# mimoralea/gym-soccer-littman94

Hardware: AMD Instinct MI355X
Metric: env-steps/sec (whole node) at batch=1M random joint actions; HBM GB/s vs peak (higher is better)
Workload: dtype int8

## Files before the change

gym_soccer_littman94_amd/_lib.py:

```python
import ctypes as C
import os

_HERE = os.path.dirname(os.path.abspath(__file__))
LIB_PATH = os.path.join(_HERE, "libsoccer_hip.so")

OK, E_INVALID, E_HIP, E_NOMEM, E_STATE = 0, -1, -2, -3, -4
F_AUTORESET = 1
F_NULL_STREAM = 2
F_HOST_MAPPED = 4
F_STEP_STATS = 8
F_STREAM_ACTIONS = 16


class SoccerHipError(RuntimeError):
    """A HIP runtime failure inside libsoccer_hip.so."""


class Config(C.Structure):
    _fields_ = [("n_lanes", C.c_uint64), ("width", C.c_int32), ("height", C.c_int32),
                ("slip_prob", C.c_double), ("max_steps", C.c_int32), ("device", C.c_int32),
                ("seed", C.c_uint64), ("lane_offset", C.c_uint64), ("flags", C.c_uint32),
                ("envs_per_thread", C.c_uint32), ("stream", C.c_void_p)]


# ... 268 lines not shown
    "soccer_comm_unique_id": (C.c_int, [C.c_void_p]),
    "soccer_comm_init": (C.c_int, [C.c_void_p, C.c_int32, C.c_int32, C.c_void_p]),
    "soccer_comm_destroy": (C.c_int, [C.c_void_p]),
    "soccer_comm_all_gather": (C.c_int, [C.c_void_p, C.c_void_p, C.c_void_p, C.c_uint64]),
    "soccer_comm_sum_u64": (C.c_int, [C.c_void_p, C.c_void_p, C.c_int32]),
    "soccer_comm_max_f64": (C.c_int, [C.c_void_p, C.c_void_p, C.c_int32]),
    "soccer_comm_barrier": (C.c_int, [C.c_void_p]),
    "soccer_malloc": (C.c_int, [C.c_void_p, C.c_size_t, C.POINTER(C.c_void_p)]),
    "soccer_free": (C.c_int, [C.c_void_p, C.c_void_p]),
    "soccer_memcpy_h2d": (C.c_int, [C.c_void_p, C.c_void_p, C.c_void_p, C.c_size_t]),
    "soccer_memcpy_d2h": (C.c_int, [C.c_void_p, C.c_void_p, C.c_void_p, C.c_size_t]),
    "soccer_memset": (C.c_int, [C.c_void_p, C.c_void_p, C.c_int, C.c_size_t]),
    "soccer_timer_start": (C.c_int, [C.c_void_p]),
    "soccer_timer_stop": (C.c_int, [C.c_void_p, C.POINTER(C.c_float)]),
    "soccer_timer_mark": (C.c_int, [C.c_void_p]),
    "soccer_timer_read": (C.c_int, [C.c_void_p, C.POINTER(C.c_float)]),
    "soccer_stamp": (C.c_int, [C.c_void_p, C.c_int32]),
    "soccer_stamps_clear": (C.c_int, [C.c_void_p, C.c_int32, C.c_int32]),
    "soccer_stamps_read": (C.c_int, [C.c_void_p, C.c_int32, C.c_int32, C.c_void_p, C.POINTER(C.c_int32)]),
    "soccer_graph_begin": (C.c_int, [C.c_void_p]),
    "soccer_graph_end": (C.c_int, [C.c_void_p, C.POINTER(C.c_void_p)]),
    "soccer_graph_launch": (C.c_int, [C.c_void_p, C.c_void_p, C.c_int32]),
    "soccer_graph_info": (C.c_int, [C.c_void_p, C.POINTER(C.c_int32), C.POINTER(C.c_int64), C.POINTER(C.c_int32)]),
    "soccer_graph_destroy": (C.c_int, [C.c_void_p, C.c_void_p]),
}

_lib = None


def _share_torch_hip_runtime():
    import importlib.util
    import sys
    if os.environ.get("SOCCER_HIP_RUNTIME", "") == "system" or "torch" in sys.modules:
        return
    try:
        spec = importlib.util.find_spec("torch")
    except Exception:
        spec = None
    if spec is None or not spec.origin:
        return
    path = os.path.join(os.path.dirname(spec.origin), "lib", "libamdhip64.so")
    if os.path.exists(path):
        try:
            C.CDLL(path, mode=C.RTLD_GLOBAL)
        except OSError:
            pass
# ... 33 lines not shown
```

gym_soccer_littman94_amd/core.py:

```python
import ctypes as C
import weakref

import numpy as np

from . import _lib
from ._device import DeviceArray, _ptr
from ._lib import Config, RolloutArgs, StepArgs
from .learners import (GradientPlay, MinimaxQLearner, MinimaxQPopulation, OpponentModelPopulation, QLearner, QPopulation,
                       RegretLearner, RegretPopulation, WolfPHCLearner, WolfPopulation, _meta_of_cross_play, league_config,
                       minimax_q_config, minimax_q_population_config, om_derive, om_model, om_population_config, q_learning_config,
                       q_population_config, regret_average, regret_learner_config, regret_policy, regret_population_config,
                       wolf_phc_config, wolf_population_config)


def meta_lds_bytes(n_a, n_b):
    stride = (n_a + n_b + 2) | 1
    return 128 + 8 * ((n_a + 2) * stride + n_a + 1) + 4 * n_a


class SoccerBatch:

    def __init__(self, n_lanes, width=5, height=4, slip_prob=0.0, seed=0, autoreset=False,
                 max_steps=100, device=0, lane_offset=0, stream=None, envs_per_thread=0, host_mapped=False, step_stats=True,
                 stream_actions=False):
# ... 561 lines not shown
        self._check(self.lib.soccer_stamps_clear(self.h, int(first), int(count)))

    def stamps(self, first=0, count=256):
        t = np.zeros(int(count), np.uint64); khz = C.c_int32()
        self._check(self.lib.soccer_stamps_read(self.h, int(first), int(count), t.ctypes.data, C.byref(khz)))
        return t, int(khz.value)

    def graph_begin(self):
        self._check(self.lib.soccer_graph_begin(self.h))

    def graph_end(self):
        g = C.c_void_p()
        self._check(self.lib.soccer_graph_end(self.h, C.byref(g)))
        return g

    def graph_launch(self, g, replays=1):
        self._check(self.lib.soccer_graph_launch(self.h, g, int(replays)))

    def graph_info(self, g):
        nodes, steps, runs = C.c_int32(), C.c_int64(), C.c_int32()
        self._check(self.lib.soccer_graph_info(g, C.byref(nodes), C.byref(steps), C.byref(runs)))
        return {"kernel_nodes": int(nodes.value), "steps_fused": int(steps.value), "fused_launches": int(runs.value)}

    def graph_destroy(self, g):
        self.lib.soccer_graph_destroy(self.h, g)
```

gym_soccer_littman94_amd/csrc/soccer_handle.hpp:

```cpp
#pragma once
#include <hip/hip_runtime.h>

#include <string>
#include <vector>

#include "../../include/soccer_hip.h"
#include "soccer_inlists.hpp"
#include "soccer_kernels.hpp"
#include "soccer_plan_io.hpp"
#include "soccer_rules.hpp"

#pragma GCC visibility push(hidden)

using namespace soccer;

int fail(soccer_handle* h, int code, const char* fmt, ...);

#define HIP_TRY(h, expr)                                                                         \
    do {                                                                                         \
        hipError_t e_ = (expr);                                                                  \
        if (e_ != hipSuccess)                                                                    \
            return fail((h), e_ == hipErrorOutOfMemory ? SOCCER_E_NOMEM : SOCCER_E_HIP,          \
                        "%s failed: %s", #expr, hipGetErrorString(e_));                          \
    } while (0)

// ... 29 lines not shown
    void release(void* p) {
        for (size_t i = 0; i < bufs.size(); ++i) if (bufs[i].ptr == p) { drop(bufs[i]); bufs.erase(bufs.begin() + i); return; }
    }
    void clear() {
        for (const Buf& b : bufs) drop(b);
        bufs.clear(); ready = false;
    }

private:
    template <class T> static size_t bytes(size_t count) { return count ? count * sizeof(T) : 1; }
    static void drop(const Buf& b) { (void)(b.pinned ? hipHostFree(b.ptr) : hipFree(b.ptr)); }
    template <class T>
    int take(soccer_handle* h, hipError_t e, bool pinned, T** out) {
        if (e != hipSuccess) {
            *out = nullptr;
            return e == hipErrorOutOfMemory ? fail(h, SOCCER_E_NOMEM, "out of %s memory for %s", pinned ? "pinned host" : "device", what)
                                            : fail(h, SOCCER_E_HIP, "allocation for %s failed: %s", what, hipGetErrorString(e));
        }
        bufs.push_back(Buf{*out, pinned});
        return SOCCER_OK;
    }
};

struct soccer_graph {
    hipGraph_t graph = nullptr;
    hipGraphExec_t exec = nullptr;
    uint64_t ticks = 0;
    int start_slot = 0;
    bool stamped = false;
    int32_t kernel_nodes = 0;
    int64_t steps_fused = 0;
    int32_t fused_launches = 0;
};

struct PendingRun {
    soccer_step_args first{};
    int64_t len = 0;
    int64_t act_stride = 0, out_stride = 0;
};

struct Learner;

struct PassBufs {
    double* buf[2] = {nullptr, nullptr};
    unsigned long long* words = nullptr;
    int32_t* done = nullptr;
    int32_t* open = nullptr;
    int stride = 0;
};
// ... 38 lines not shown
    unsigned long long* d_hist = nullptr;
    unsigned int* d_misuse = nullptr;
    unsigned int* misuse_host = nullptr;
    uint8_t* d_state = nullptr;
    size_t state_stride = 0;
    int state_streams = 6;
    uint8_t* stage_dev = nullptr;
    uint8_t* stage_host = nullptr;
    bool mapped = false;
    size_t stage_bytes = 0;
    int tick_slot = 0;
    uint64_t tick = 0;
    bool slip = false, lut_lds = false;
    size_t smem_bytes = 0;
    int E = 4;
    int grid_cap = 2048;
    bool capturing = false;
    uint64_t capture_ticks = 0;
    int capture_calls = 0;
    int capture_start_slot = 0;
    PendingRun run;
    bool graph_fuse = true;
    int capture_kernels = 0;
    int64_t capture_steps_fused = 0; int capture_fused_launches = 0;
    int n_cu = 256;
    size_t lds_limit = 64 * 1024;
    uint4* d_sub = nullptr;
    uint4* rec_host = nullptr; uint4* rec_dev = nullptr; uint32_t rec_seq = 0;
    swar::Consts swar_c{}; bool swar_ok = false;
    swar::SlipConsts slip_c{}; bool slip_swar_ok = false;
    uint32_t* d_slip_lut = nullptr;
    uint32_t* d_slip_step_lut = nullptr;
    size_t hist_slots = kHistSlots;
    bool timer_stamped = false; int wall_clock_khz = 100000;
    bool capture_stamped = false;
    bool stamp_poll = false;
    unsigned long long stamp_prev = 0;
    unsigned long long swar_launch_lanes = kSwarLaunchLanes;
    int rollout_pref = 0;
    soccer_rollout_shape_info last_rollout{};
    SlipF64* d_slip_f64 = nullptr;
    uint32_t* d_worklist = nullptr;
    unsigned long long* d_traj_hist = nullptr;
    void* comm = nullptr; int comm_world = 0, comm_rank = 0;
    unsigned long long* d_comm_scratch = nullptr;
    PlanIO plan{};
// ... 27 lines not shown
    size_t mg_need[5] = {0, 0, 0, 0, 0};
    OwnedBufs mg_bufs{"the meta-game solver"};
    std::vector<Learner*> learners;
    std::string err;

    soccer_handle() = default;
    soccer_handle(const soccer_handle&) = delete;
    soccer_handle& operator=(const soccer_handle&) = delete;
    ~soccer_handle();
};

constexpr size_t kStampStride = 8;
constexpr size_t kMappedBytes = 64 + 8 * kStampStride * SOCCER_STAMP_SLOTS;

static inline void bind_tick(soccer_handle* h, KernelParams& P, uint64_t ticks) {
    P.tick_in = h->d_tick + (h->tick_slot ? 16 : 0);
    P.tick_out = h->d_tick + (h->tick_slot ? 0 : 16);
    h->tick_slot ^= 1;
    if (h->capturing) { h->capture_ticks += ticks; h->capture_calls += 1; }
    else h->tick += ticks;
}

static inline void note_kernel(soccer_handle* h) { if (h->capturing) h->capture_kernels += 1; }

static inline int grid_for(const soccer_handle* h, uint64_t work_items) {
    uint64_t blocks = (work_items + kBlock - 1) / kBlock;
    if (blocks < 1) blocks = 1;
    if (blocks > (uint64_t)h->grid_cap) blocks = h->grid_cap;
    return static_cast<int>(blocks);
}

hipError_t rollout_raise_smem_limit(const soccer_handle* h, size_t bytes);
int rollout_enqueue(soccer_handle* h, const soccer_rollout_args* a, const soccer_rollout_extra* x, unsigned long long* hist);
int flush_run(soccer_handle* h);
static inline int flush_pending(soccer_handle* h) { return h->run.len ? flush_run(h) : SOCCER_OK; }
void comm_release(soccer_handle* h);
void learners_release(soccer_handle* h);
void gradient_players_release(soccer_handle* h);
constexpr int kMinimaxBatch = 16;
int minimax_check(soccer_handle* h, const char* what, double gamma);
int minimax_prepare(soccer_handle* h);
int response_rows(soccer_handle* h, const char* what, const char* name, int n, const double* pol);
int response_upload(soccer_handle* h, double* dst, const double* pol, int n, hipMemcpyKind kind = hipMemcpyHostToDevice);

#pragma GCC visibility pop
```

gym_soccer_littman94_amd/csrc/soccer_hip.hip:

```cpp
#include <hip/hip_runtime.h>

#include <algorithm>
#include <atomic>
#include <chrono>
#include <cstdarg>
#include <cstdio>
#include <cstdlib>
#include <cstring>
#include <memory>
#include <string>
#include <vector>

#include "soccer_dispatch.hpp"
#include "soccer_handle.hpp"
#include "soccer_env_kernels.hpp"
#include "soccer_slip.hpp"

static thread_local std::string g_err;

int fail(soccer_handle* h, int code, const char* fmt, ...) {
    char buf[512];
    va_list ap; va_start(ap, fmt); vsnprintf(buf, sizeof buf, fmt, ap); va_end(ap);
    if (h) h->err = buf; else g_err = buf;
    return code;
// ... 125 lines not shown
        }
        if (ST.lut_step_ok && !std::getenv("SOCCER_STEP_SLIP_ONE_BY_ONE")) {
            std::vector<uint32_t> img(kSlipStepLdsWords, 0xFFFFFFFFu);
            std::memcpy(img.data(), ST.lut_step, kSlipStepBuckets);
            std::memcpy(img.data() + kSlipStepBuckets / 4, ST.T, sizeof(ST.T));
            if (int rc = h->bufs.alloc(nullptr, img.size(), &h->d_slip_step_lut)) return rc;
            HIP_TRY(nullptr, hipMemcpy(h->d_slip_step_lut, img.data(), img.size() * sizeof(uint32_t), hipMemcpyHostToDevice));
        }
        {
            const SlipF64 F = make_slip_f64(ST);
            if (int rc = h->bufs.alloc(nullptr, 1, &h->d_slip_f64)) return rc;
            HIP_TRY(nullptr, hipMemcpy(h->d_slip_f64, &F, sizeof F, hipMemcpyHostToDevice));
        }
        h->slip_c = swar::SlipConsts{};
        for (int i = 0; i < 9; ++i) h->slip_c.CB[i] = ST.CB[i];
        h->slip_c.c_off = ST.c_off;
    }
    set_key(h, cfg->seed);
    h->swar_ok = swar::fits(R.H, R.W, cfg->max_steps);
    if (h->swar_ok) h->swar_c = swar::make_consts(R.H, R.W, R.goal_lo, R.goal_hi, cfg->max_steps, R.n_isd, R.isd, P.autoreset != 0u);
    h->slip = cfg->slip_prob != 0.0;
    if (const char* e2 = std::getenv("SOCCER_ROLLOUT")) h->rollout_pref = std::atoi(e2);
    if (const char* e4 = std::getenv("SOCCER_GRAPH_FUSE")) h->graph_fuse = std::atoi(e4) != 0;
    if (const char* e3 = std::getenv("SOCCER_SWAR_LAUNCH_LANES")) {
        const unsigned long long v = std::strtoull(e3, nullptr, 10) & ~3ull;
        if (v >= 4ull && v <= kSwarLaunchLanes) h->swar_launch_lanes = v;
    }
    h->E = e ? static_cast<int>(e) : 4;

    const size_t nc_bytes = (R.next_cell.size() + kIsdWords) * sizeof(uint32_t);
    const size_t lut_bytes = R.lut.size() * sizeof(uint16_t);
    if (nc_bytes > 150 * 1024)
        return fail(nullptr, SOCCER_E_INVALID, "pitch too large: the move/bounds table (%zu bytes) must fit the 160 KB LDS", nc_bytes);
    if (int rc = h->bufs.alloc(nullptr, R.lut.size(), &h->d_lut)) return rc;
    HIP_TRY(nullptr, hipMemcpy(h->d_lut, R.lut.data(), lut_bytes, hipMemcpyHostToDevice));
    P.lut = h->d_lut; P.lut_len = static_cast<int32_t>(R.lut.size());
    h->lut_lds = nc_bytes + lut_bytes <= 150 * 1024;
    h->smem_bytes = nc_bytes + (h->lut_lds ? lut_bytes : 0);
    if (h->smem_bytes > 48 * 1024) {
        const size_t b = h->smem_bytes;
        hipError_t se = rollout_raise_smem_limit(h, b);
        if (se == hipSuccess)
            se = with_shape(h, [&](auto slip, auto lds) {
                return hipFuncSetAttribute(reinterpret_cast<const void*>(&reset_kernel<decltype(lds)::value, decltype(slip)::value>),
                                           hipFuncAttributeMaxDynamicSharedMemorySize, (int)b);
            });
// ... 46 lines not shown
    unsigned long long slots[32] = {0};
    slots[0] = tick; slots[16] = tick;
    HIP_TRY(h, hipMemcpy(h->d_tick, slots, sizeof slots, hipMemcpyHostToDevice));
    h->tick = tick;
    return SOCCER_OK;
}
extern "C" uint64_t soccer_get_seed(const soccer_handle* h) { return h ? h->cfg.seed : 0; }

extern "C" int batched_reset(soccer_handle* h, const uint8_t* mask, const double* u_reset, uint16_t* obs) {
    if (!h) return fail(nullptr, SOCCER_E_INVALID, "handle is NULL");
    if (!aligned(u_reset, 8) || !aligned(obs, 2))
        return fail(h, SOCCER_E_INVALID, "batched_reset: u_reset must be 8-byte and obs 2-byte aligned");
    HIP_TRY(h, hipSetDevice(h->cfg.device));
    if (int rc = flush_pending(h)) return rc;
    KernelParams P = h->P;
    bind_tick(h, P, 1);
    ResetIO io{mask, u_reset, obs};
    const ResetPlan R = plan_reset(handle_facts(h), ResetCall{mask != nullptr, u_reset != nullptr, aligned(mask, 4) && aligned(obs, 8)});
    const unsigned long long n4 = R.n4;
    if (n4) {
        ResetSwar RS{h->swar_c, P.state, P.state_stride, P.state_layout, n4, P.lane_offset, P.tick_in, P.tick_out, P.key0, P.key1, mask, obs};
        const dim3 g(static_cast<unsigned>(((n4 >> 2) + kBlock - 1) / kBlock)), b(kBlock);
        with_flag(R.masked, [&](auto masked) { with_flag(R.slip, [&](auto slip) {
            hipLaunchKernelGGL((reset_kernel_swar<decltype(masked)::value, decltype(slip)::value>), g, b, 0, h->stream, RS);
        }); });
        note_kernel(h);
    }
    if (n4 < P.n) {
        KernelParams Q = P;
        Q.first = n4; Q.n = P.n - n4;
        if (n4) Q.tick_out = nullptr;
        const dim3 g(grid_for(h, Q.n)), b(kBlock);
        with_flag(R.lut_lds, [&](auto lds) { with_flag(R.slip, [&](auto slip) {
            hipLaunchKernelGGL((reset_kernel<decltype(lds)::value, decltype(slip)::value>), g, b, h->smem_bytes, h->stream, Q, io);
        }); });
        note_kernel(h);
    }
    HIP_TRY(h, hipGetLastError());
    return SOCCER_OK;
}

static int fetch_state(soccer_handle* h, std::vector<uint8_t>& img) {
    const size_t n = h->P.n, S = h->state_stride, bytes = (size_t)h->state_streams * S;
    if (h->mapped) std::memcpy(img.data(), h->d_state, bytes);
    else HIP_TRY(h, hipMemcpy(img.data(), h->d_state, bytes, hipMemcpyDeviceToHost));
    if (h->state_streams == 3) {
        for (size_t i = 0; i < n; ++i) {
            swar::Group G;
            swar::unpack3(img[i], img[S + i], img[2 * S + i], G);
            img[5 * S + i] = (uint8_t)G.tt; img[4 * S + i] = (uint8_t)G.ps; img[3 * S + i] = (uint8_t)G.cb;
            img[2 * S + i] = (uint8_t)G.rb; img[S + i] = (uint8_t)G.ca; img[i] = (uint8_t)G.ra;
        }
    }
    return SOCCER_OK;
}

extern "C" int soccer_state_streams(const soccer_handle* h) { return h ? h->state_streams : 0; }
// ... 347 lines not shown
    if (hist) {
        std::vector<unsigned long long> shards(h->hist_slots * kHistStride);
        HIP_TRY(h, hipMemcpy(shards.data(), h->d_hist, shards.size() * sizeof(unsigned long long), hipMemcpyDeviceToHost));
        hist[0] = hist[1] = hist[2] = 0;
        for (size_t s = 0; s < h->hist_slots; ++s) for (int b = 0; b < 3; ++b) hist[b] += shards[s * kHistStride + b];
    }
    if (misuse) {
        const volatile unsigned int* m = h->misuse_host;
        *misuse = (m[0] ? 1u : 0u) | (m[1] ? 2u : 0u) | (m[2] ? 4u : 0u);
    }
    return SOCCER_OK;
}

extern "C" uint32_t soccer_peek_misuse(const soccer_handle* h) {
    if (!h || !h->misuse_host) return 0u;
    const volatile unsigned int* m = h->misuse_host;
    return (m[0] ? SOCCER_MISUSE_FROZEN : 0u) | (m[1] ? SOCCER_MISUSE_ACTION : 0u) | (m[2] ? SOCCER_MISUSE_OBSERVATION : 0u);
}

extern "C" int soccer_reset_stats(soccer_handle* h) {
    if (!h) return fail(nullptr, SOCCER_E_INVALID, "handle is NULL");
    HIP_TRY(h, hipSetDevice(h->cfg.device));
    if (int rc = flush_pending(h)) return rc;
    HIP_TRY(h, hipMemsetAsync(h->d_hist, 0, sizeof(unsigned long long) * h->hist_slots * kHistStride, h->stream));
    HIP_TRY(h, hipMemsetAsync(h->d_misuse, 0, 64, h->stream));
    return SOCCER_OK;
}

extern "C" int soccer_malloc(soccer_handle* h, size_t bytes, void** dptr) {
    if (!h || !dptr) return fail(h, SOCCER_E_INVALID, "handle/dptr is NULL");
    HIP_TRY(h, hipSetDevice(h->cfg.device));
    HIP_TRY(h, hipMalloc(dptr, bytes ? bytes : 1));
    return SOCCER_OK;
}
extern "C" int soccer_free(soccer_handle* h, void* dptr) {
    if (!h) return fail(nullptr, SOCCER_E_INVALID, "handle is NULL");
    HIP_TRY(h, hipSetDevice(h->cfg.device));
    if (dptr) HIP_TRY(h, hipFree(dptr));
    return SOCCER_OK;
}
extern "C" int soccer_memcpy_h2d(soccer_handle* h, void* dst, const void* src, size_t bytes) {
    if (!h) return fail(nullptr, SOCCER_E_INVALID, "handle is NULL");
    if (h->capturing) return fail(h, SOCCER_E_STATE, "soccer_memcpy_h2d during graph capture");
    HIP_TRY(h, hipSetDevice(h->cfg.device));
    HIP_TRY(h, hipMemcpyAsync(dst, src, bytes, hipMemcpyHostToDevice, h->stream));
    HIP_TRY(h, hipStreamSynchronize(h->stream));
    return SOCCER_OK;
}
extern "C" int soccer_memcpy_d2h(soccer_handle* h, void* dst, const void* src, size_t bytes) {
    if (!h) return fail(nullptr, SOCCER_E_INVALID, "handle is NULL");
    if (h->capturing) return fail(h, SOCCER_E_STATE, "soccer_memcpy_d2h during graph capture");
    HIP_TRY(h, hipSetDevice(h->cfg.device));
    HIP_TRY(h, hipMemcpyAsync(dst, src, bytes, hipMemcpyDeviceToHost, h->stream));
    HIP_TRY(h, hipStreamSynchronize(h->stream));
    return SOCCER_OK;
}
extern "C" int soccer_memset(soccer_handle* h, void* dst, int value, size_t bytes) {
    if (!h) return fail(nullptr, SOCCER_E_INVALID, "handle is NULL");
    HIP_TRY(h, hipSetDevice(h->cfg.device));
    if (int rc = flush_pending(h)) return rc;
    HIP_TRY(h, hipMemsetAsync(dst, value, bytes, h->stream));
    return SOCCER_OK;
}

__global__ void stamp_kernel(unsigned long long* slot) {
    if (threadIdx.x == 0) *slot = wall_clock64();
}

static volatile unsigned long long* stamp_host(soccer_handle* h) {
    return reinterpret_cast<volatile unsigned long long*>(reinterpret_cast<uint8_t*>(h->misuse_host) + 64);
}
static unsigned long long* stamp_dev(soccer_handle* h) {
    return reinterpret_cast<unsigned long long*>(reinterpret_cast<uint8_t*>(h->d_misuse) + 64);
}

extern "C" int soccer_stamp(soccer_handle* h, int32_t slot) {
    if (!h) return fail(nullptr, SOCCER_E_INVALID, "handle is NULL");
    if (slot < 0 || slot >= SOCCER_STAMP_SLOTS) return fail(h, SOCCER_E_INVALID, "stamp slot %d out of range (0..%d)", slot, SOCCER_STAMP_SLOTS - 1);
    HIP_TRY(h, hipSetDevice(h->cfg.device));
    if (int rc = flush_pending(h)) return rc;
    hipLaunchKernelGGL(stamp_kernel, dim3(1), dim3(64), 0, h->stream, stamp_dev(h) + kStampStride * slot);
    HIP_TRY(h, hipGetLastError());
    return SOCCER_OK;
}

extern "C" int soccer_stamps_clear(soccer_handle* h, int32_t first, int32_t count) {
    if (!h) return fail(nullptr, SOCCER_E_INVALID, "handle is NULL");
    if (first < 0 || count < 0 || first + count > SOCCER_STAMP_SLOTS) return fail(h, SOCCER_E_INVALID, "stamp range out of bounds");
    for (int32_t i = 0; i < count; ++i) stamp_host(h)[kStampStride * (first + i)] = 0ull;
    std::atomic_thread_fence(std::memory_order_seq_cst);
    return SOCCER_OK;
}

extern "C" int soccer_stamps_read(soccer_handle* h, int32_t first, int32_t count, uint64_t* ticks, int32_t* khz) {
    if (!h) return fail(nullptr, SOCCER_E_INVALID, "handle is NULL");
    if (first < 0 || count < 0 || first + count > SOCCER_STAMP_SLOTS || (count && !ticks)) return fail(h, SOCCER_E_INVALID, "stamp range out of bounds");
    for (int32_t i = 0; i < count; ++i) ticks[i] = stamp_host(h)[kStampStride * (first + i)];
    if (khz) *khz = h->wall_clock_khz;
    return SOCCER_OK;
}

extern "C" int soccer_timer_start(soccer_handle* h) {
    if (!h) return fail(nullptr, SOCCER_E_INVALID, "handle is NULL");
// ... 54 lines not shown
        __builtin_ia32_pause();
    }
    (void)hipGetLastError();
    HIP_TRY(h, hipEventElapsedTime(elapsed_ms, h->ev0, h->ev1));
    return SOCCER_OK;
}
extern "C" int soccer_timer_stop(soccer_handle* h, float* elapsed_ms) {
    if (int rc = soccer_timer_mark(h)) return rc;
    return soccer_timer_read(h, elapsed_ms);
}

__global__ void move_tick_kernel(unsigned long long* dst, const unsigned long long* src) {
    if (threadIdx.x == 0) *dst = *src;
}

extern "C" int soccer_graph_begin(soccer_handle* h) {
    if (!h) return fail(nullptr, SOCCER_E_INVALID, "handle is NULL");
    if (h->capturing) return fail(h, SOCCER_E_STATE, "graph capture already in progress");
    HIP_TRY(h, hipSetDevice(h->cfg.device));
    HIP_TRY(h, hipStreamBeginCapture(h->stream, hipStreamCaptureModeThreadLocal));
    h->capturing = true; h->capture_ticks = 0; h->capture_calls = 0; h->capture_stamped = false;
    h->capture_start_slot = h->tick_slot;
    h->run = PendingRun{}; h->capture_kernels = 0; h->capture_steps_fused = 0; h->capture_fused_launches = 0;
    return SOCCER_OK;
}

extern "C" int soccer_graph_end(soccer_handle* h, soccer_graph** out) {
    if (!h || !out) return fail(h, SOCCER_E_INVALID, "handle/out is NULL");
    if (!h->capturing) return fail(h, SOCCER_E_STATE, "no graph capture in progress");
    if (const int rc = flush_pending(h)) {
        const std::string why = h->err;
        hipGraph_t dead = nullptr;
        h->capturing = false; h->tick_slot = h->capture_start_slot;
        (void)hipStreamEndCapture(h->stream, &dead);
        if (dead) (void)hipGraphDestroy(dead);
        (void)hipGetLastError();
        h->err = why;
        return rc;
    }
    if (h->capture_calls % 2 != 0) {
        hipLaunchKernelGGL(move_tick_kernel, dim3(1), dim3(64), 0, h->stream,
                           h->d_tick + (h->capture_start_slot ? 16 : 0), h->d_tick + (h->tick_slot ? 16 : 0));
        h->tick_slot = h->capture_start_slot;
    }
    h->capturing = false;
    hipGraph_t graph = nullptr;
    HIP_TRY(h, hipStreamEndCapture(h->stream, &graph));
    soccer_graph* g = new soccer_graph();
    g->kernel_nodes = h->capture_kernels; g->steps_fused = h->capture_steps_fused; g->fused_launches = h->capture_fused_launches;
    g->graph = graph; g->ticks = h->capture_ticks; g->start_slot = h->capture_start_slot; g->stamped = h->capture_stamped;
    hipError_t e = hipGraphInstantiate(&g->exec, graph, nullptr, nullptr, 0);
    if (e != hipSuccess) {
        (void)hipGraphDestroy(graph); delete g;
        return fail(h, SOCCER_E_HIP, "hipGraphInstantiate failed: %s", hipGetErrorString(e));
    }
    (void)hipGraphUpload(g->exec, h->stream);
    (void)hipGetLastError();
    *out = g;
    return SOCCER_OK;
}

extern "C" int soccer_graph_launch(soccer_handle* h, soccer_graph* g, int32_t replays) {
    if (!h || !g) return fail(h, SOCCER_E_INVALID, "handle/graph is NULL");
    if (h->capturing) return fail(h, SOCCER_E_STATE, "soccer_graph_launch during graph capture");
    HIP_TRY(h, hipSetDevice(h->cfg.device));
    if (replays > 0 && h->tick_slot != g->start_slot) {
        HIP_TRY(h, hipMemcpyAsync(h->d_tick + (g->start_slot ? 16 : 0), h->d_tick + (h->tick_slot ? 16 : 0),
                                  sizeof(unsigned long long), hipMemcpyDeviceToDevice, h->stream));
        h->tick_slot = g->start_slot;
    }
    h->stamp_poll = replays == 1 && g->stamped && hipStreamQuery(h->stream) == hipSuccess;
    (void)hipGetLastError();
    h->timer_stamped = g->stamped;
    if (h->stamp_poll) h->stamp_prev = stamp_host(h)[kStampStride];
    for (int32_t r = 0; r < replays; ++r) HIP_TRY(h, hipGraphLaunch(g->exec, h->stream));
    h->tick += g->ticks * (uint64_t)(replays > 0 ? replays : 0);
    return SOCCER_OK;
}

extern "C" int soccer_graph_info(const soccer_graph* g, int32_t* kernel_nodes, int64_t* steps_fused, int32_t* fused_launches) {
    if (!g) return fail(nullptr, SOCCER_E_INVALID, "graph is NULL");
    if (kernel_nodes) *kernel_nodes = g->kernel_nodes;
    if (steps_fused) *steps_fused = g->steps_fused;
    if (fused_launches) *fused_launches = g->fused_launches;
    return SOCCER_OK;
}

extern "C" int soccer_graph_destroy(soccer_handle* h, soccer_graph* g) {
    if (!g) return SOCCER_OK;
    if (h) { (void)hipSetDevice(h->cfg.device); (void)hipStreamSynchronize(h->stream); }
    if (g->exec) (void)hipGraphExecDestroy(g->exec);
    if (g->graph) (void)hipGraphDestroy(g->graph);
    delete g;
    return SOCCER_OK;
}

extern "C" int soccer_trajectory_returns(soccer_handle* h, int32_t n_steps, const int8_t* reward, const uint8_t* terminated,
                                         const uint8_t* truncated, int64_t stride, int8_t* last_return,
                                         int32_t* episode_count, uint64_t hist[3]) {
    if (!h) return fail(nullptr, SOCCER_E_INVALID, "handle is NULL");
    if (h->capturing) return fail(h, SOCCER_E_STATE, "soccer_trajectory_returns during graph capture");
    if (n_steps < 1 || !reward || !terminated || !truncated)
        return fail(h, SOCCER_E_INVALID, "soccer_trajectory_returns: n_steps >= 1 and the reward / terminated / truncated trajectories are required");
    if (stride < (int64_t)h->P.n) return fail(h, SOCCER_E_INVALID, "soccer_trajectory_returns: stride must be >= n_lanes");
    if (!aligned(episode_count, 4)) return fail(h, SOCCER_E_INVALID, "soccer_trajectory_returns: episode_count must be 4-byte aligned");
    HIP_TRY(h, hipSetDevice(h->cfg.device));
    const size_t slots = (size_t)h->grid_cap * 2;
// ... 28 lines not shown
```

gym_soccer_littman94_amd/csrc/soccer_launch_plan.hpp:

```cpp
#pragma once
#include <cstddef>
#include <cstdint>

#include "../../include/soccer_hip.h"

namespace soccer {

struct HandleFacts {
    bool swar_ok, slip, slip_swar_ok;
    bool slip_lut, slip_step_lut;
    bool small, wide;
    bool lut_lds;
    bool policy_a, policy_b, step_stats, slip_int_one, stream_actions;
    bool capturing, worklist;
    int E, rollout_pref, nS;
    unsigned lane_phase;
    size_t smem_bytes, lds_limit;
    unsigned long long n;
};

struct StepCall {
    bool dword_io;
    bool u_step, u_reset, u_aligned16;
    bool last_return, last_return_aligned4;
// ... 143 lines not shown
    sh.full = R.full ? 1 : 0;
    sh.table_placement = R.table_placement;
    sh.parts = R.swar ? parts : 1; sh.chunks = chunks;
    sh.dynamic_lds_bytes = R.smem;
    return sh;
}

struct ResetCall {
    bool mask, u_reset, dword_io;
};

struct ResetPlan {
    unsigned long long n4;
    bool masked, slip, lut_lds;
};

inline ResetPlan plan_reset(const HandleFacts& f, const ResetCall& c) {
    ResetPlan R{};
    if (f.swar_ok && !c.u_reset && f.E != 1 && f.lane_phase == 0u && c.dword_io) R.n4 = f.n & ~3ull;
    R.masked = c.mask; R.slip = f.slip; R.lut_lds = f.lut_lds;
    return R;
}

}
```

gym_soccer_littman94_amd/csrc/soccer_rollout.hip:

```cpp
#include <hip/hip_runtime.h>

#include <algorithm>

#include "soccer_dispatch.hpp"
#include "soccer_handle.hpp"
#include "soccer_rollout_kernels.hpp"
#include "soccer_slip.hpp"

static_assert(kSlipLutWords == kSlipLdsWords, "table layout shared with the kernels");
static_assert(kPlanBlock == kBlock && kPlanSlipLutBytes == kSlipLutWords * sizeof(uint32_t), "the plan sizes LDS as the kernels use it");

hipError_t rollout_raise_smem_limit(const soccer_handle* h, size_t bytes) {
    hipError_t se = hipSuccess;
    for (int e : {1, 4, 8})
        for (bool d : {false, true})
            if (se == hipSuccess)
                se = with_value<1, 4, 8>(e, [&](auto ev) { return with_flag(d, [&](auto dyn) { return with_shape(h, [&](auto slip, auto lds) {
                    return hipFuncSetAttribute(reinterpret_cast<const void*>(&rollout_kernel<decltype(ev)::value, decltype(slip)::value, decltype(lds)::value, decltype(dyn)::value>),
                                               hipFuncAttributeMaxDynamicSharedMemorySize, (int)bytes);
                }); }); });
    return se;
}

static int launch_rollout(soccer_handle* h, const RolloutPlan& R, int E, const KernelParams& P, const RolloutIO& io) {
    const dim3 g(grid_for(h, (P.n + E - 1) / E)), b(kBlock);
    const bool launched =
    with_value<8, 4, 1>(E, [&](auto ev) { return
    with_flag(R.slip, [&](auto slip) { return
    with_flag(R.lut_lds, [&](auto lds) { return
    with_flag(R.dyn, [&](auto dv) {
        hipLaunchKernelGGL((rollout_kernel<decltype(ev)::value, decltype(slip)::value, decltype(lds)::value, decltype(dv)::value>), g, b, h->smem_bytes, h->stream, P, io);
        return true;
    }); }); }); });
    if (!launched) return NOT_COMPILED(h, "rollout_kernel");
    note_kernel(h);
    return SOCCER_OK;
}

static int launch_rollout_swar(soccer_handle* h, const RolloutPlan& R, dim3 g, const RolloutSwar& RS, const RolloutIO& io) {
    hipError_t se = hipSuccess;
    const bool launched =
    with_value<0, 1, 2, 3, 4, 5>(R.dm, [&](auto dv) { return
    with_value<0, 1, 2>(R.sm, [&](auto sv) { return
    with_value<0, 1>(R.geo, [&](auto gv) { return
    with_flag(R.full, [&](auto fv) { return
    with_flag(R.stats, [&](auto tv) {
        constexpr int DM = decltype(dv)::value, SM = decltype(sv)::value, GEO = decltype(gv)::value;
        constexpr bool FULL = decltype(fv)::value, STATS = decltype(tv)::value;
        constexpr bool compiled = STATS || kUnreadShape<DM, FULL>;
        if constexpr (compiled) {
            if (R.smem > 48 * 1024)
                se = hipFuncSetAttribute(reinterpret_cast<const void*>(&rollout_swar_kernel<DM, SM, GEO, FULL, STATS>), hipFuncAttributeMaxDynamicSharedMemorySize, (int)R.smem);
            if (se == hipSuccess) hipLaunchKernelGGL((rollout_swar_kernel<DM, SM, GEO, FULL, STATS>), g, dim3(kBlock), R.smem, h->stream, RS, io);
        }
        return compiled;
    }); }); }); }); });
    if (!launched) return NOT_COMPILED(h, "rollout_swar_kernel");
    if (se != hipSuccess)
        return fail(h, se == hipErrorOutOfMemory ? SOCCER_E_NOMEM : SOCCER_E_HIP, "hipFuncSetAttribute(rollout_swar_kernel, %zu bytes of dynamic LDS) failed: %s",
                    R.smem, hipGetErrorString(se));
    note_kernel(h);
    return SOCCER_OK;
}

extern "C" int batched_rollout(soccer_handle* h, const soccer_rollout_args* a) { return batched_rollout_ex(h, a, nullptr); }

extern "C" int soccer_rollout_shape(const soccer_handle* h, soccer_rollout_shape_info* out) {
    if (!h || !out) return SOCCER_E_INVALID;
    *out = h->last_rollout;
    out->lds_limit = h->lds_limit;
    return SOCCER_OK;
}

extern "C" int batched_rollout_ex(soccer_handle* h, const soccer_rollout_args* a, const soccer_rollout_extra* x) {
    if (!h) return fail(nullptr, SOCCER_E_INVALID, "handle is NULL");
    if (int rc = flush_pending(h)) return rc;
// ... 67 lines not shown
```

gym_soccer_littman94_amd/csrc/soccer_step.hip:

```cpp
#include <hip/hip_runtime.h>

#include <algorithm>

#include "soccer_dispatch.hpp"
#include "soccer_handle.hpp"
#include "soccer_step_kernels.hpp"

static inline size_t worklist_count_word(const soccer_handle* h) { return ((size_t)(h->P.n >> 2) + 5) & ~(size_t)1; }
static inline uint32_t* worklist_count(const soccer_handle* h) { return h->d_worklist ? h->d_worklist + worklist_count_word(h) : nullptr; }
static bool ensure_worklist(soccer_handle* h) {
    if (h->d_worklist) return true;
    const size_t words = worklist_count_word(h) + 2 + 4;
    if (h->bufs.alloc(h, words, &h->d_worklist) != SOCCER_OK) { (void)hipGetLastError(); return false; }
    if (hipMemsetAsync(h->d_worklist, 0, words * sizeof(uint32_t), h->stream) != hipSuccess) {
        (void)hipGetLastError(); h->bufs.release(h->d_worklist); h->d_worklist = nullptr; return false;
    }
    return true;
}

static int launch_step(soccer_handle* h, const KernelParams& P, const StepIO& io, const StepLaunch& L) {
    const dim3 b(kBlock);
    const unsigned long long* tick_in = h->capturing ? P.tick_in : nullptr;
    const unsigned long long tick = (unsigned long long)(h->tick - 1);
    if (L.family == kStepSwar) {
// ... 1 lines not shown
        for (unsigned long long c0 = P.first; c0 < P.first + P.n; c0 += h->swar_launch_lanes) {
            const unsigned long long cn = std::min<unsigned long long>(h->swar_launch_lanes, P.first + P.n - c0);
            const bool last = c0 + cn == P.first + P.n;
            const dim3 gh(static_cast<unsigned>(((cn >> 2) + kBlock - 1) / kBlock));
            SwarParams Q{h->swar_c, P.key0, P.key1, P.lane_offset + c0, last ? P.tick_out : nullptr, P.misuse,
                         off(io.obs, c0), off(io.reward, c0), off(io.terminated, c0), off(io.truncated, c0),
                         off(io.reward_a_f32, c0), off(io.reward_b_f32, c0), off(io.finished, c0), off(io.last_return, c0),
                         off(io.prob_code, c0), off(io.final_obs, c0),
                         P.step_stats ? P.hist : nullptr, P.hist_mask,
                         h->slip_c, reinterpret_cast<const swar::Quad*>(P.sub), h->d_slip_step_lut,
                         P.policy_a, P.policy_b, off(io.u_step, c0), off(io.u_reset, c0),
                         h->d_slip_f64, h->d_worklist, worklist_count(h)};
            const bool launched =
            with_value<0, 1, 2>(L.out, [&](auto ov) { return
            with_value<0, 1, 2, 3>(L.slipm, [&](auto sv) { return
            with_flag(L.policy, [&](auto pv) { return
            with_value<0, 1>(L.geo, [&](auto gv) { return
            with_flag(L.expl, [&](auto xv) { return
            with_flag(L.wide, [&](auto wv) {
                constexpr int OUT = decltype(ov)::value, SLIPM = decltype(sv)::value, GEO = decltype(gv)::value;
                constexpr bool POLICY = decltype(pv)::value, EXPL = decltype(xv)::value, WIDE = decltype(wv)::value;
                constexpr bool compiled = (SLIPM == 3 ? EXPL : (!EXPL || SLIPM == 0)) && !(WIDE && GEO == 1);
                if constexpr (compiled)
                    hipLaunchKernelGGL((step_kernel_swar<OUT, SLIPM, POLICY, GEO, EXPL, WIDE ? kStateWide : kStatePacked>), gh, b, 0, h->stream,
                                       P.state + c0, P.state_stride, off(io.act_a, c0), off(io.act_b, c0), tick_in, cn | act_stream, tick, Q);
                return compiled;
            }); }); }); }); }); });
            if (!launched) return NOT_COMPILED(h, "step_kernel_swar");
            note_kernel(h);
            if (L.exact_tail) {
                KernelParams R = P; R.first = c0; R.n = cn; R.tick_out = nullptr;
                StepIO jo = io; jo.worklist = h->d_worklist; jo.work_count = worklist_count(h);
                hipLaunchKernelGGL((step_kernel<true, true, true, true>), dim3(1), b, 0, h->stream, R, jo);
                note_kernel(h);
            }
        }
    } else if (L.family == kStepHot) {
        const dim3 gh(static_cast<unsigned>(((P.n >> 2) + kBlock - 1) / kBlock));
        const bool launched =
        with_flag(L.slip, [&](auto slip) { return
        with_flag(L.int_only, [&](auto int_only) {
            constexpr bool compiled = decltype(slip)::value || !decltype(int_only)::value;
            if constexpr (compiled)
                hipLaunchKernelGGL((step_kernel_hot<decltype(slip)::value, decltype(int_only)::value>), gh, b, 0, h->stream,
                                   P.state, P.state_stride, io.act_a, io.act_b, tick_in, P.n, tick, P, io);
            return compiled;
        }); });
        if (!launched) return NOT_COMPILED(h, "step_kernel_hot");
        note_kernel(h);
    } else {
        const dim3 g(grid_for(h, (P.n + 3) / 4));
        const bool launched =
        with_flag(L.slip, [&](auto slip) { return
        with_flag(L.explicit_u, [&](auto explicit_u) { return
        with_flag(L.vec, [&](auto vec) { return
        with_flag(L.shared, [&](auto shared) {
            constexpr bool EXPLICIT_U = decltype(explicit_u)::value, VEC = decltype(vec)::value, SHARED = decltype(shared)::value;
            constexpr bool compiled = VEC ? (SHARED || !EXPLICIT_U) : !SHARED;
            if constexpr (compiled)
                hipLaunchKernelGGL((step_kernel<decltype(slip)::value, EXPLICIT_U, VEC, SHARED>), g, b, 0, h->stream, P, io);
            return compiled;
        }); }); }); });
        if (!launched) return NOT_COMPILED(h, "step_kernel");
        note_kernel(h);
    }
    return SOCCER_OK;
}

static StepCall step_call(const soccer_step_args* a) {
    StepCall c;
    c.dword_io = aligned(a->act_a, 4) && aligned(a->act_b, 4) && aligned(a->reward, 4) &&
                 aligned(a->terminated, 4) && aligned(a->truncated, 4) && aligned(a->prob_code, 4) &&
                 aligned(a->obs, 8) && aligned(a->final_obs, 8) && aligned(a->reward_a_f32, 16) && aligned(a->reward_b_f32, 16) &&
                 aligned(a->finished, 4);
    c.u_step = a->u_step; c.u_reset = a->u_reset; c.u_aligned16 = aligned(a->u_step, 16) && aligned(a->u_reset, 16);
    c.last_return = a->last_return; c.last_return_aligned4 = aligned(a->last_return, 4);
    c.full = a->prob_code || a->final_obs; c.gym = a->reward_a_f32 || a->reward_b_f32 || a->finished;
    return c;
}

static int launch_one_step(soccer_handle* h, const soccer_step_args* a) {
    HandleFacts f = handle_facts(h);
    const StepCall c = step_call(a);
// ... 131 lines not shown
```

include/soccer_hip.h:

```cpp
#ifndef SOCCER_HIP_H
#define SOCCER_HIP_H

#include <stddef.h>
#include <stdint.h>

#ifdef __cplusplus
extern "C" {
#endif

#define SOCCER_ABI_VERSION 3

#define SOCCER_OK            0
#define SOCCER_E_INVALID    -1
#define SOCCER_E_HIP        -2
#define SOCCER_E_NOMEM      -3
#define SOCCER_E_STATE      -4

#define SOCCER_F_AUTORESET   1u
#define SOCCER_F_NULL_STREAM 2u
#define SOCCER_F_STEP_STATS  8u
#define SOCCER_F_HOST_MAPPED 4u
#define SOCCER_F_STREAM_ACTIONS 16u

#define SOCCER_NOOP  0
// ... 507 lines not shown
int soccer_comm_all_gather(soccer_handle* h, const void* send, void* recv, uint64_t bytes_per_rank);
int soccer_comm_sum_u64(soccer_handle* h, uint64_t* values, int32_t count);
int soccer_comm_max_f64(soccer_handle* h, double* values, int32_t count);
int soccer_comm_barrier(soccer_handle* h);

int soccer_malloc(soccer_handle* h, size_t bytes, void** dptr);
int soccer_free(soccer_handle* h, void* dptr);
int soccer_memcpy_h2d(soccer_handle* h, void* dst, const void* src, size_t bytes);
int soccer_memcpy_d2h(soccer_handle* h, void* dst, const void* src, size_t bytes);
int soccer_memset(soccer_handle* h, void* dst, int value, size_t bytes);
int soccer_timer_start(soccer_handle* h);
int soccer_timer_mark(soccer_handle* h);
int soccer_timer_read(soccer_handle* h, float* elapsed_ms);
int soccer_timer_stop(soccer_handle* h, float* elapsed_ms);
#define SOCCER_STAMP_SLOTS 256
int soccer_stamp(soccer_handle* h, int32_t slot);
int soccer_stamps_clear(soccer_handle* h, int32_t first, int32_t count);
int soccer_stamps_read(soccer_handle* h, int32_t first, int32_t count, uint64_t* ticks, int32_t* khz);

int soccer_graph_begin(soccer_handle* h);
int soccer_graph_end(soccer_handle* h, soccer_graph** out);
int soccer_graph_launch(soccer_handle* h, soccer_graph* g, int32_t replays);
int soccer_graph_info(const soccer_graph* g, int32_t* kernel_nodes, int64_t* steps_fused, int32_t* fused_launches);
int soccer_graph_destroy(soccer_handle* h, soccer_graph* g);

#ifdef __cplusplus
}
#endif
#endif
```

Before: 788.2 billion.

## Replay single-call captured graphs as direct recorded kernel launches

During graph capture, each step/reset/rollout kernel launch is recorded as a host closure that can be relaunched with fresh tick pointers. When a capture holds exactly one call with no memsets, stamps or worklist kernels, graph_end drops the HIP graph and replay relaunches the recorded kernels directly on the stream, alternating tick slots. This avoids graph-launch overhead, the move_tick node and the device-to-device tick copy on slot mismatch. The trade-off is a std::function per launch, a different replay path enabled by default (SOCCER_GRAPH_DIRECT), and the risk that the tick/stamp state handling differs from the graph path.

Result: no change. 789.5 billion, median of 2 (+0.2%).

```diff
diff --git a/gym_soccer_littman94_amd/_lib.py b/gym_soccer_littman94_amd/_lib.py
--- a/gym_soccer_littman94_amd/_lib.py
+++ b/gym_soccer_littman94_amd/_lib.py
@@ -314,6 +314,7 @@
     "soccer_graph_end": (C.c_int, [C.c_void_p, C.POINTER(C.c_void_p)]),
     "soccer_graph_launch": (C.c_int, [C.c_void_p, C.c_void_p, C.c_int32]),
     "soccer_graph_info": (C.c_int, [C.c_void_p, C.POINTER(C.c_int32), C.POINTER(C.c_int64), C.POINTER(C.c_int32)]),
+    "soccer_graph_replay_info": (C.c_int, [C.c_void_p, C.POINTER(C.c_int32), C.POINTER(C.c_int32), C.POINTER(C.c_int32)]),
     "soccer_graph_destroy": (C.c_int, [C.c_void_p, C.c_void_p]),
 }
 
diff --git a/gym_soccer_littman94_amd/core.py b/gym_soccer_littman94_amd/core.py
--- a/gym_soccer_littman94_amd/core.py
+++ b/gym_soccer_littman94_amd/core.py
@@ -607,5 +607,10 @@
         self._check(self.lib.soccer_graph_info(g, C.byref(nodes), C.byref(steps), C.byref(runs)))
         return {"kernel_nodes": int(nodes.value), "steps_fused": int(steps.value), "fused_launches": int(runs.value)}
 
+    def graph_replay_info(self, g):
+        direct, launches, extra = C.c_int32(), C.c_int32(), C.c_int32()
+        self._check(self.lib.soccer_graph_replay_info(g, C.byref(direct), C.byref(launches), C.byref(extra)))
+        return {"direct": bool(direct.value), "launches_per_replay": int(launches.value), "extra_nodes": int(extra.value)}
+
     def graph_destroy(self, g):
         self.lib.soccer_graph_destroy(self.h, g)
diff --git a/gym_soccer_littman94_amd/csrc/soccer_handle.hpp b/gym_soccer_littman94_amd/csrc/soccer_handle.hpp
--- a/gym_soccer_littman94_amd/csrc/soccer_handle.hpp
+++ b/gym_soccer_littman94_amd/csrc/soccer_handle.hpp
@@ -1,6 +1,7 @@
 #pragma once
 #include <hip/hip_runtime.h>
 
+#include <functional>
 #include <string>
 #include <vector>
 
@@ -76,9 +77,17 @@
     }
 };
 
+struct LaunchRecord {
+    std::function<void(hipStream_t, const unsigned long long* tick_in, unsigned long long* tick_out)> launch;
+    bool publishes;
+};
+
 struct soccer_graph {
     hipGraph_t graph = nullptr;
     hipGraphExec_t exec = nullptr;
+    bool direct = false;
+    bool move_node = false;
+    std::vector<LaunchRecord> records;
     uint64_t ticks = 0;
     int start_slot = 0;
     bool stamped = false;
@@ -163,6 +172,9 @@
     PendingRun run;
     bool graph_fuse = true;
     int capture_kernels = 0;
+    std::vector<LaunchRecord> capture_records;
+    bool capture_other = false;
+    bool graph_direct = true;
     int64_t capture_steps_fused = 0; int capture_fused_launches = 0;
     int n_cu = 256;
     size_t lds_limit = 64 * 1024;
@@ -236,6 +248,13 @@
 }
 
 static inline void note_kernel(soccer_handle* h) { if (h->capturing) h->capture_kernels += 1; }
+static inline void note_other(soccer_handle* h) { if (h->capturing) h->capture_other = true; }
+
+template <class F>
+static inline void launch_recorded(soccer_handle* h, const unsigned long long* tick_in, unsigned long long* tick_out, F&& launch) {
+    launch(h->stream, tick_in, tick_out);
+    if (h->capturing) h->capture_records.push_back(LaunchRecord{launch, tick_out != nullptr});
+}
 
 static inline int grid_for(const soccer_handle* h, uint64_t work_items) {
     uint64_t blocks = (work_items + kBlock - 1) / kBlock;
diff --git a/gym_soccer_littman94_amd/csrc/soccer_hip.hip b/gym_soccer_littman94_amd/csrc/soccer_hip.hip
--- a/gym_soccer_littman94_amd/csrc/soccer_hip.hip
+++ b/gym_soccer_littman94_amd/csrc/soccer_hip.hip
@@ -171,6 +171,7 @@
     h->slip = cfg->slip_prob != 0.0;
     if (const char* e2 = std::getenv("SOCCER_ROLLOUT")) h->rollout_pref = std::atoi(e2);
     if (const char* e4 = std::getenv("SOCCER_GRAPH_FUSE")) h->graph_fuse = std::atoi(e4) != 0;
+    if (const char* e5 = std::getenv("SOCCER_GRAPH_DIRECT")) h->graph_direct = std::atoi(e5) != 0;
     if (const char* e3 = std::getenv("SOCCER_SWAR_LAUNCH_LANES")) {
         const unsigned long long v = std::strtoull(e3, nullptr, 10) & ~3ull;
         if (v >= 4ull && v <= kSwarLaunchLanes) h->swar_launch_lanes = v;
@@ -263,7 +264,10 @@
         ResetSwar RS{h->swar_c, P.state, P.state_stride, P.state_layout, n4, P.lane_offset, P.tick_in, P.tick_out, P.key0, P.key1, mask, obs};
         const dim3 g(static_cast<unsigned>(((n4 >> 2) + kBlock - 1) / kBlock)), b(kBlock);
         with_flag(R.masked, [&](auto masked) { with_flag(R.slip, [&](auto slip) {
-            hipLaunchKernelGGL((reset_kernel_swar<decltype(masked)::value, decltype(slip)::value>), g, b, 0, h->stream, RS);
+            launch_recorded(h, RS.tick_in, RS.tick_out, [=](hipStream_t s, const unsigned long long* tin, unsigned long long* tout) {
+                ResetSwar rs = RS; rs.tick_in = tin; rs.tick_out = tout;
+                hipLaunchKernelGGL((reset_kernel_swar<decltype(masked)::value, decltype(slip)::value>), g, b, 0, s, rs);
+            });
         }); });
         note_kernel(h);
     }
@@ -273,7 +277,10 @@
         if (n4) Q.tick_out = nullptr;
         const dim3 g(grid_for(h, Q.n)), b(kBlock);
         with_flag(R.lut_lds, [&](auto lds) { with_flag(R.slip, [&](auto slip) {
-            hipLaunchKernelGGL((reset_kernel<decltype(lds)::value, decltype(slip)::value>), g, b, h->smem_bytes, h->stream, Q, io);
+            launch_recorded(h, Q.tick_in, Q.tick_out, [=, smem = h->smem_bytes](hipStream_t s, const unsigned long long* tin, unsigned long long* tout) {
+                KernelParams q = Q; q.tick_in = tin; q.tick_out = tout;
+                hipLaunchKernelGGL((reset_kernel<decltype(lds)::value, decltype(slip)::value>), g, b, smem, s, q, io);
+            });
         }); });
         note_kernel(h);
     }
@@ -667,6 +674,7 @@
     if (!h) return fail(nullptr, SOCCER_E_INVALID, "handle is NULL");
     HIP_TRY(h, hipSetDevice(h->cfg.device));
     if (int rc = flush_pending(h)) return rc;
+    note_other(h);
     HIP_TRY(h, hipMemsetAsync(h->d_hist, 0, sizeof(unsigned long long) * h->hist_slots * kHistStride, h->stream));
     HIP_TRY(h, hipMemsetAsync(h->d_misuse, 0, 64, h->stream));
     return SOCCER_OK;
@@ -704,6 +712,7 @@
     if (!h) return fail(nullptr, SOCCER_E_INVALID, "handle is NULL");
     HIP_TRY(h, hipSetDevice(h->cfg.device));
     if (int rc = flush_pending(h)) return rc;
+    note_other(h);
     HIP_TRY(h, hipMemsetAsync(dst, value, bytes, h->stream));
     return SOCCER_OK;
 }
@@ -724,6 +733,7 @@
     if (slot < 0 || slot >= SOCCER_STAMP_SLOTS) return fail(h, SOCCER_E_INVALID, "stamp slot %d out of range (0..%d)", slot, SOCCER_STAMP_SLOTS - 1);
     HIP_TRY(h, hipSetDevice(h->cfg.device));
     if (int rc = flush_pending(h)) return rc;
+    note_other(h);
     hipLaunchKernelGGL(stamp_kernel, dim3(1), dim3(64), 0, h->stream, stamp_dev(h) + kStampStride * slot);
     HIP_TRY(h, hipGetLastError());
     return SOCCER_OK;
@@ -824,6 +834,7 @@
     h->capturing = true; h->capture_ticks = 0; h->capture_calls = 0; h->capture_stamped = false;
     h->capture_start_slot = h->tick_slot;
     h->run = PendingRun{}; h->capture_kernels = 0; h->capture_steps_fused = 0; h->capture_fused_launches = 0;
+    h->capture_records.clear(); h->capture_other = false;
     return SOCCER_OK;
 }
 
@@ -834,23 +845,36 @@
         const std::string why = h->err;
         hipGraph_t dead = nullptr;
         h->capturing = false; h->tick_slot = h->capture_start_slot;
+        h->capture_records.clear();
         (void)hipStreamEndCapture(h->stream, &dead);
         if (dead) (void)hipGraphDestroy(dead);
         (void)hipGetLastError();
         h->err = why;
         return rc;
     }
-    if (h->capture_calls % 2 != 0) {
+    const ReplayPlan R = plan_replay(ReplayFacts{h->capture_calls, (int)h->capture_records.size(),
+                                                 h->capture_other || (int)h->capture_records.size() != h->capture_kernels, h->graph_direct});
+    if (R.move_node) {
         hipLaunchKernelGGL(move_tick_kernel, dim3(1), dim3(64), 0, h->stream,
                            h->d_tick + (h->capture_start_slot ? 16 : 0), h->d_tick + (h->tick_slot ? 16 : 0));
-        h->tick_slot = h->capture_start_slot;
-    }
+    }
+    h->tick_slot = h->capture_start_slot;
     h->capturing = false;
+    std::vector<LaunchRecord> records;
+    records.swap(h->capture_records);
     hipGraph_t graph = nullptr;
     HIP_TRY(h, hipStreamEndCapture(h->stream, &graph));
     soccer_graph* g = new soccer_graph();
     g->kernel_nodes = h->capture_kernels; g->steps_fused = h->capture_steps_fused; g->fused_launches = h->capture_fused_launches;
-    g->graph = graph; g->ticks = h->capture_ticks; g->start_slot = h->capture_start_slot; g->stamped = h->capture_stamped;
+    g->ticks = h->capture_ticks; g->start_slot = h->capture_start_slot; g->stamped = h->capture_stamped;
+    g->direct = R.direct; g->move_node = R.move_node;
+    if (R.direct) {
+        if (graph) (void)hipGraphDestroy(graph);
+        g->records = std::move(records);
+        *out = g;
+        return SOCCER_OK;
+    }
+    g->graph = graph;
     hipError_t e = hipGraphInstantiate(&g->exec, graph, nullptr, nullptr, 0);
     if (e != hipSuccess) {
         (void)hipGraphDestroy(graph); delete g;
@@ -866,6 +890,17 @@
     if (!h || !g) return fail(h, SOCCER_E_INVALID, "handle/graph is NULL");
     if (h->capturing) return fail(h, SOCCER_E_STATE, "soccer_graph_launch during graph capture");
     HIP_TRY(h, hipSetDevice(h->cfg.device));
+    if (g->direct) {
+        h->stamp_poll = false; h->timer_stamped = false;
+        for (int32_t r = 0; r < replays; ++r) {
+            const unsigned long long* tick_in = h->d_tick + (h->tick_slot ? 16 : 0);
+            unsigned long long* tick_out = h->d_tick + (h->tick_slot ? 0 : 16);
+            for (const LaunchRecord& rec : g->records) rec.launch(h->stream, tick_in, rec.publishes ? tick_out : nullptr);
+            HIP_TRY(h, hipGetLastError());
+            h->tick_slot ^= 1; h->tick += g->ticks;
+        }
+        return SOCCER_OK;
+    }
     if (replays > 0 && h->tick_slot != g->start_slot) {
         HIP_TRY(h, hipMemcpyAsync(h->d_tick + (g->start_slot ? 16 : 0), h->d_tick + (h->tick_slot ? 16 : 0),
                                   sizeof(unsigned long long), hipMemcpyDeviceToDevice, h->stream));
@@ -885,6 +920,14 @@
     if (kernel_nodes) *kernel_nodes = g->kernel_nodes;
     if (steps_fused) *steps_fused = g->steps_fused;
     if (fused_launches) *fused_launches = g->fused_launches;
+    return SOCCER_OK;
+}
+
+extern "C" int soccer_graph_replay_info(const soccer_graph* g, int32_t* direct, int32_t* launches_per_replay, int32_t* extra_nodes) {
+    if (!g) return fail(nullptr, SOCCER_E_INVALID, "graph is NULL");
+    if (direct) *direct = g->direct ? 1 : 0;
+    if (launches_per_replay) *launches_per_replay = g->direct ? (int32_t)g->records.size() : 1;
+    if (extra_nodes) *extra_nodes = g->move_node ? 1 : 0;
     return SOCCER_OK;
 }
 
diff --git a/gym_soccer_littman94_amd/csrc/soccer_launch_plan.hpp b/gym_soccer_littman94_amd/csrc/soccer_launch_plan.hpp
--- a/gym_soccer_littman94_amd/csrc/soccer_launch_plan.hpp
+++ b/gym_soccer_littman94_amd/csrc/soccer_launch_plan.hpp
@@ -189,4 +189,25 @@
     return R;
 }
 
-}
+struct ReplayFacts {
+    int calls;
+    int launches;
+    bool other;
+    bool direct_enabled;
+};
+
+struct ReplayPlan {
+    bool direct;
+    bool move_node;
+    int launches_per_replay;
+};
+
+inline ReplayPlan plan_replay(const ReplayFacts& f) {
+    ReplayPlan R{};
+    R.direct = f.direct_enabled && f.calls == 1 && f.launches >= 1 && !f.other;
+    R.move_node = !R.direct && f.calls % 2 != 0;
+    R.launches_per_replay = R.direct ? f.launches : 1;
+    return R;
+}
+
+}
diff --git a/gym_soccer_littman94_amd/csrc/soccer_rollout.hip b/gym_soccer_littman94_amd/csrc/soccer_rollout.hip
--- a/gym_soccer_littman94_amd/csrc/soccer_rollout.hip
+++ b/gym_soccer_littman94_amd/csrc/soccer_rollout.hip
@@ -29,7 +29,10 @@
     with_flag(R.slip, [&](auto slip) { return
     with_flag(R.lut_lds, [&](auto lds) { return
     with_flag(R.dyn, [&](auto dv) {
-        hipLaunchKernelGGL((rollout_kernel<decltype(ev)::value, decltype(slip)::value, decltype(lds)::value, decltype(dv)::value>), g, b, h->smem_bytes, h->stream, P, io);
+        launch_recorded(h, P.tick_in, P.tick_out, [=, smem = h->smem_bytes](hipStream_t s, const unsigned long long* tin, unsigned long long* tout) {
+            KernelParams p = P; p.tick_in = tin; p.tick_out = tout;
+            hipLaunchKernelGGL((rollout_kernel<decltype(ev)::value, decltype(slip)::value, decltype(lds)::value, decltype(dv)::value>), g, b, smem, s, p, io);
+        });
         return true;
     }); }); }); });
     if (!launched) return NOT_COMPILED(h, "rollout_kernel");
@@ -51,7 +54,11 @@
         if constexpr (compiled) {
             if (R.smem > 48 * 1024)
                 se = hipFuncSetAttribute(reinterpret_cast<const void*>(&rollout_swar_kernel<DM, SM, GEO, FULL, STATS>), hipFuncAttributeMaxDynamicSharedMemorySize, (int)R.smem);
-            if (se == hipSuccess) hipLaunchKernelGGL((rollout_swar_kernel<DM, SM, GEO, FULL, STATS>), g, dim3(kBlock), R.smem, h->stream, RS, io);
+            if (se == hipSuccess)
+                launch_recorded(h, RS.tick_in, RS.tick_out, [=, smem = R.smem](hipStream_t s, const unsigned long long* tin, unsigned long long* tout) {
+                    RolloutSwar rs = RS; rs.tick_in = tin; rs.tick_out = tout;
+                    hipLaunchKernelGGL((rollout_swar_kernel<DM, SM, GEO, FULL, STATS>), g, dim3(kBlock), smem, s, rs, io);
+                });
         }
         return compiled;
     }); }); }); }); });
diff --git a/gym_soccer_littman94_amd/csrc/soccer_step.hip b/gym_soccer_littman94_amd/csrc/soccer_step.hip
--- a/gym_soccer_littman94_amd/csrc/soccer_step.hip
+++ b/gym_soccer_littman94_amd/csrc/soccer_step.hip
@@ -47,8 +47,11 @@
                 constexpr bool POLICY = decltype(pv)::value, EXPL = decltype(xv)::value, WIDE = decltype(wv)::value;
                 constexpr bool compiled = (SLIPM == 3 ? EXPL : (!EXPL || SLIPM == 0)) && !(WIDE && GEO == 1);
                 if constexpr (compiled)
-                    hipLaunchKernelGGL((step_kernel_swar<OUT, SLIPM, POLICY, GEO, EXPL, WIDE ? kStateWide : kStatePacked>), gh, b, 0, h->stream,
-                                       P.state + c0, P.state_stride, off(io.act_a, c0), off(io.act_b, c0), tick_in, cn | act_stream, tick, Q);
+                    launch_recorded(h, tick_in, Q.tick_out, [=](hipStream_t s, const unsigned long long* tin, unsigned long long* tout) {
+                        SwarParams q = Q; q.tick_out = tout;
+                        hipLaunchKernelGGL((step_kernel_swar<OUT, SLIPM, POLICY, GEO, EXPL, WIDE ? kStateWide : kStatePacked>), gh, b, 0, s,
+                                           P.state + c0, P.state_stride, off(io.act_a, c0), off(io.act_b, c0), tin, cn | act_stream, tick, q);
+                    });
                 return compiled;
             }); }); }); }); }); });
             if (!launched) return NOT_COMPILED(h, "step_kernel_swar");
@@ -58,6 +61,7 @@
                 StepIO jo = io; jo.worklist = h->d_worklist; jo.work_count = worklist_count(h);
                 hipLaunchKernelGGL((step_kernel<true, true, true, true>), dim3(1), b, 0, h->stream, R, jo);
                 note_kernel(h);
+                note_other(h);
             }
         }
     } else if (L.family == kStepHot) {
@@ -67,8 +71,11 @@
         with_flag(L.int_only, [&](auto int_only) {
             constexpr bool compiled = decltype(slip)::value || !decltype(int_only)::value;
             if constexpr (compiled)
-                hipLaunchKernelGGL((step_kernel_hot<decltype(slip)::value, decltype(int_only)::value>), gh, b, 0, h->stream,
-                                   P.state, P.state_stride, io.act_a, io.act_b, tick_in, P.n, tick, P, io);
+                launch_recorded(h, tick_in, P.tick_out, [=](hipStream_t s, const unsigned long long* tin, unsigned long long* tout) {
+                    KernelParams p = P; p.tick_out = tout;
+                    hipLaunchKernelGGL((step_kernel_hot<decltype(slip)::value, decltype(int_only)::value>), gh, b, 0, s,
+                                       p.state, p.state_stride, io.act_a, io.act_b, tin, p.n, tick, p, io);
+                });
             return compiled;
         }); });
         if (!launched) return NOT_COMPILED(h, "step_kernel_hot");
@@ -83,7 +90,10 @@
             constexpr bool EXPLICIT_U = decltype(explicit_u)::value, VEC = decltype(vec)::value, SHARED = decltype(shared)::value;
             constexpr bool compiled = VEC ? (SHARED || !EXPLICIT_U) : !SHARED;
             if constexpr (compiled)
-                hipLaunchKernelGGL((step_kernel<decltype(slip)::value, EXPLICIT_U, VEC, SHARED>), g, b, 0, h->stream, P, io);
+                launch_recorded(h, P.tick_in, P.tick_out, [=](hipStream_t s, const unsigned long long* tin, unsigned long long* tout) {
+                    KernelParams p = P; p.tick_in = tin; p.tick_out = tout;
+                    hipLaunchKernelGGL((step_kernel<decltype(slip)::value, EXPLICIT_U, VEC, SHARED>), g, b, 0, s, p, io);
+                });
             return compiled;
         }); }); }); });
         if (!launched) return NOT_COMPILED(h, "step_kernel");
diff --git a/include/soccer_hip.h b/include/soccer_hip.h
--- a/include/soccer_hip.h
+++ b/include/soccer_hip.h
@@ -553,6 +553,7 @@
 int soccer_graph_end(soccer_handle* h, soccer_graph** out);
 int soccer_graph_launch(soccer_handle* h, soccer_graph* g, int32_t replays);
 int soccer_graph_info(const soccer_graph* g, int32_t* kernel_nodes, int64_t* steps_fused, int32_t* fused_launches);
+int soccer_graph_replay_info(const soccer_graph* g, int32_t* direct, int32_t* launches_per_replay, int32_t* extra_nodes);
 int soccer_graph_destroy(soccer_handle* h, soccer_graph* g);
 
 #ifdef __cplusplus
```
